# argsim/argsim

Measured on AMD Instinct MI355X. Metric: sentences/sec per ELBO step, higher is better.
Workload: dtype f32; 1 GPU; BASELINE configs[1]: 1xMI355X fp32, latent_dim 128, vocab 8k, seq_len 64, batch 256 per GPU; FULL synthetic Zipf batches, dim_emb 512, 3 layers, step 20000; global_batch=256, seq_len=64, parallelism=dp1, gru=persistent

## Files before the change

argsim_amd/csrc/kernels.h:

```cpp
#pragma once
#include <hip/hip_runtime.h>
#include <stdint.h>

#include "gemm_plan.h"

namespace avae {

struct GemmArgs {
    const float* A; const float* B; float* C; const float* bias;
    int M, N, K, lda, ldb, ldc;
    float alpha;
    int accumulate;
    int split_k;
    const int* dyn; int dyn_kind;
    int dyn_expect;
    int thin;
    const float* A2; const float* B2; float* C2; const float* bias2;
    float* slab = nullptr; size_t slab_floats = 0;
    unsigned short* c16 = nullptr;
    int nt8 = 1;
};
hipError_t gemm_f32(hipStream_t st, bool a_mc, bool b_nc, const GemmArgs& g);
hipError_t gemm_f32s(hipStream_t st, bool a_mc, bool b_nc, const GemmArgs& g);
hipError_t gemm_bf16_direct(hipStream_t st, bool a_mc, bool b_nc, const GemmArgs& g);
// ... 100 lines not shown
hipError_t embed_scatter_add2(hipStream_t st, float* dE, const int32_t* ids0, const float* dout0, int n0, const int32_t* ids1,
                              const float* dout1, int n1, int D, int V, int32_t* scratch);
bool id_groups_supported(int V);
inline size_t id_groups_ints(size_t n, size_t V) { return 4 * V + 2 + n + (n / 32 + V + 1) + 2 * V + 4; }
hipError_t id_groups_build(hipStream_t st, const int32_t* ids, int n, int V, int32_t* scratch, bool lists);
const int32_t* id_groups_rank(int32_t* scratch, int n, int V);
const int32_t* id_groups_uid(int32_t* scratch, int n, int V);
const int32_t* id_groups_count(int32_t* scratch, int n, int V);
hipError_t rank_rows(hipStream_t st, int32_t* out, const int32_t* ids, const int32_t* rank, int n, int V);
hipError_t rows_gather_ranked(hipStream_t st, float* dst, const float* src, const int32_t* ids, const int32_t* rank, int n, int W, int V);
hipError_t rows_group_sum(hipStream_t st, float* dst, const int32_t* ids, const float* src, int n, int W, int V, int32_t* scratch);
hipError_t rows_add_indexed(hipStream_t st, float* dst, const float* src, const int32_t* uid, const int32_t* nuniq, int n_max, int D);
inline size_t embed_scatter_scratch_ints(size_t n, size_t V) { return 4 * V + 2 + n + (n / 32 + V + 1); }
struct RowOrder { const int32_t* lens; int add, T, cpj; int32_t* perm; int32_t* slens; };
hipError_t row_order(hipStream_t st, const RowOrder* orders, int n, int Breal, int B, int S, int32_t* steps_sum = nullptr, int sum_rows = 0);
hipError_t rows_gather(hipStream_t st, float* dst, const float* src, const int32_t* idx, const int32_t* n_dev, int n_max, int D, const int32_t* map = nullptr);
hipError_t rows_expand(hipStream_t st, float* dst, const float* src, const int32_t* rank, int rows, int D, const int32_t* map = nullptr);
hipError_t pick_last(hipStream_t st, float* h, const float* hs, const int32_t* lens, int B, int W, const int32_t* map = nullptr);
hipError_t pick_last16(hipStream_t st, float* h, const unsigned short* hs16, const int32_t* lens, int B, int W, const int32_t* map = nullptr);
hipError_t pick_last_add(hipStream_t st, float* dhs, const float* d, const int32_t* lens, int B, int W, const int32_t* map = nullptr);
hipError_t row_map(hipStream_t st, const int32_t* lens, int add, int S, int B, int32_t* map, int32_t* nact, int32_t* count);
hipError_t zero_rows_dyn(hipStream_t st, float* X, const int32_t* count, int rows_max, int W);
hipError_t pick_last_bwd(hipStream_t st, float* dhs, const float* dh, const int32_t* lens, int S, int B, int W);

hipError_t latent_fwd(hipStream_t st, const float* mu, const float* lv, const float* eps_in, float* eps_out, float* z,
                      float* kld, int n, int train, uint64_t seed, float free_bits, float* acc);
hipError_t latent_bwd(hipStream_t st, const float* dz, const float* mu, const float* lv, const float* eps_used,
                      float* dmu, float* dlv, int B, int R, float coef, float free_bits);

struct CeArgs {
// ... 117 lines not shown
```

argsim_amd/csrc/model.cpp:

```cpp
#include "../../include/argsim_vae.h"
#include "kernels.h"

#include <fcntl.h>
#include <sys/file.h>
#include <unistd.h>

#include <algorithm>
#include <cmath>
#include <cstdio>
#include <cstring>
#include <string>
#include <vector>

using namespace avae;

namespace {

struct ParamEntry {
    std::string name;
    int64_t offset;
    int ndim;
    int64_t shape[4];
    int g16;
    int bucket;
// ... 12 lines not shown
    std::string err;
    std::vector<ParamEntry> params;
    int64_t numel = 0;
    std::vector<std::pair<int64_t, int64_t>> buckets;
    float *P = nullptr, *G = nullptr, *M = nullptr, *Vv = nullptr;
    int64_t step = 0;
    avae_grad_hook hook = nullptr; void* hook_user = nullptr;
    std::vector<int> hook_pending;
    int persistent = 1;
    bool first_step_checked = false;
    int gru_ablate = 0, gru_force_slow = 0, gru_stagger = 0, gru_item = 2;
    int skinny = 1;
    int score_plan[4] = {0, 0, 0, 0};
    const int* expect_ptr[3] = {nullptr, nullptr, nullptr}; int expect_val[3] = {0, 0, 0};
    int compact = 2;
    int skip_pad = 1;
    int shared_device = 0; int lock_fd = -1;
    int dyn_split = 1;
    int dyn_thin = 1;
    int enc_top1 = 1;
    int table_l1 = 1;
    int bf16_act = 1;
    int bf16_sv = 1;
    int bf16_tn = 1;
    int logits16 = 1;
    int bf16_nt8 = 1;
    int bf16_direct = 0;
    int gru_spec = 2;
    int bwd_rs = 2;
    int knn_chunk = 0;
// ... 75 lines not shown
    float *xlast, *gib, *svb, *dgib, *dghb, *dxl;
    float *hc, *ho, *logits;
    float *loss_samp, *errt_samp;
    float *dho, *dhc, *dhd[2], *dgi_d, *dgh_d, *dh0, *carry, *dh0sum, *dz, *dmu, *dlv, *dhpick;
    float *dhs[2], *dgi_e, *dgh_e, *demb_src, *demb_tgt;
    std::vector<unsigned short*> e_hs16, d_hd16, e_hp16[2], d_hp16;
    std::vector<char> act_e, act_d, acth_e, acth_d;
    std::vector<unsigned short*> x16_e, x16_d;
    const unsigned short* x16_kept_e(int i) const { return x16_valid ? x16_e[i] : nullptr; }
    const unsigned short* x16_kept_d(int i) const { return x16_valid ? x16_d[i] : nullptr; }
    bool x16_valid = false;
    unsigned short *dgi16_d, *dgh16_d, *dgi16_e, *dgh16_e;
    int32_t* scat;
    int32_t *grp_src, *grp_tgt;
    int32_t *tokrow_src, *tokrow_tgt;
    float* xbuf; size_t xbuf_floats;
    int32_t *ord_perm[3], *ord_slens[3]; int ord_T[3], ord_cpj[3]; bool ord_ok[3];
    int32_t *map_src, *nact_src, *nsrc; bool compact;
    int32_t *map_tgt, *nact_tgt, *ntgt; bool compact_d;
    int Bx;
    int bx_enc() const { return compact ? Bx : 0; }
    int bx_dec() const { return compact_d ? Bx : 0; }
};

struct Bump {
    char* base; size_t off = 0;
    template <class T> T* take(size_t n) {
        off = (off + 255) & ~(size_t)255;
        T* p = base ? reinterpret_cast<T*>(base + off) : nullptr;
        off += n * sizeof(T);
// ... 11 lines not shown
    return rows >= h->cfg.dim_tgt || (rows >= 1024 && phantom_batch(h, B));
}

void layout(avae_ctx* h, Bump& b, Ws& w, int B, int Ss, int St, bool train)
{
    const int D = h->cfg.dim_emb, V = h->cfg.dim_tgt, R = h->cfg.dim_rep, L = h->cfg.rnn_layers;
    const size_t T = St + 1, rs = (size_t)Ss * B, rt = T * B;
    w.src_tm = b.take<int32_t>(rs); w.lens_src = b.take<int32_t>(B); w.lens_tgt = b.take<int32_t>(B);
    w.lead = b.take<int32_t>(rt); w.gold = b.take<int32_t>(rt); w.rank = b.take<int32_t>(rt);
    w.cidx = b.take<int32_t>(rt); w.ntok = b.take<int32_t>(4 + kPrepChunks); w.pred = b.take<int32_t>(rt);
    w.emb_src = b.take<float>(rs * D); w.emb_tgt = b.take<float>(rt * D);
    const bool tab_s = use_table(h, (int)rs, B), tab_t = use_table(h, (int)rt, B);
    w.ew = b.take<float>(tab_s ? (size_t)V * 6 * D : (tab_t ? (size_t)V * 3 * D : 0));
    w.grp_src = b.take<int32_t>(tab_s ? id_groups_ints(rs, V) : 0); w.grp_tgt = b.take<int32_t>(tab_t ? id_groups_ints(rt, V) : 0);
    w.tokrow_src = b.take<int32_t>(tab_s ? rs : 0); w.tokrow_tgt = b.take<int32_t>(tab_t ? rt : 0);
    w.e_gi.resize(L); w.e_hs.resize(L);
    for (int d = 0; d < 2; ++d) { w.e_sv[d].resize(L); w.e_hp[d].resize(L); }
    w.d_gi.resize(L); w.d_hd.resize(L); w.d_sv.resize(L); w.d_hp.resize(L);
    w.e_hs16.assign(L, nullptr); w.d_hd16.assign(L, nullptr); w.e_hp16[0].assign(L, nullptr); w.e_hp16[1].assign(L, nullptr); w.d_hp16.assign(L, nullptr);
    w.act_e.assign(L, 0); w.act_d.assign(L, 0); w.acth_e.assign(L, 0); w.acth_d.assign(L, 0);
    if (train && h->cfg.compute_dtype == 1 && h->bf16_act && h->bf16_tn && D % 8 == 0)
        for (int i = 0; i < L; ++i) {
            w.e_hs16[i] = b.take<unsigned short>(rs * 2 * D); w.e_hp16[0][i] = b.take<unsigned short>(rs * D); w.e_hp16[1][i] = b.take<unsigned short>(rs * D);
            if (i < L - 1) w.d_hd16[i] = b.take<unsigned short>(rt * D);
            w.d_hp16[i] = b.take<unsigned short>(rt * D);
        }
    w.x16_e.assign(L, nullptr); w.x16_d.assign(L, nullptr);
    w.x16_valid = train && h->cfg.compute_dtype == 1 && h->bf16_tn && !h->bf16_direct && D % 8 == 0;
    if (w.x16_valid)
        for (int i = 1; i < L; ++i) { w.x16_e[i] = b.take<unsigned short>(rs * 2 * D); w.x16_d[i] = b.take<unsigned short>(rt * D); }
// ... 310 lines not shown
{
    if (h->gru_spec != 2) return h->gru_spec;
    return expected_fill(h) < 0.60 ? 1 : 0;
}

static void gru_common(avae_ctx* h, const Ws& w, GruArgs& a, int njobs, int S, int B, int ldg, int ldh, const int32_t* lens, int Bx)
{
    const int D = h->cfg.dim_emb;
    a.njobs = njobs; a.S = S; a.B = B; a.D = D; a.ldg = ldg; a.ldh = ldh; a.lens = lens;
    a.Bx = Bx;
    gru_geometry(D, njobs, B, &a.G, &a.rows_per_group);
    a.p_begin = 0; a.p_end = S; a.counters = h->counters; a.err = h->errw; a.ablate = h->gru_ablate; a.force_slow = h->gru_force_slow;
    a.bf16 = h->cfg.compute_dtype == 1 && h->gru_bf16; a.stagger = h->gru_stagger; a.item_pipeline = h->gru_item;
    a.xbuf = w.xbuf; a.xbuf_floats = w.xbuf_floats; a.stamps = reinterpret_cast<unsigned long long*>(h->errw + 16); a.bwd_rs = h->bwd_rs != 0;
}
int build_row_orders(avae_ctx* h, Ws& w, int B, int Ss, int T, bool with_dec, bool with_enc = true)
{
    if (!h->skip_pad || !h->persistent || w.Bx % 16) return 0;
    if (w.Bx != B && !h->compact) return 0;
    const int D = h->cfg.dim_emb;
    RowOrder ord[3]; int n = 0, which[3];
    auto want = [&](int k, int njobs, int S, int ldg, int ldh, const int32_t* lens, int add) {
        GruArgs a{};
        gru_common(h, w, a, njobs, S, B, ldg, ldh, lens, w.Bx);
        const GruPlan p = gru_plan(a, true, true);
        if (p.form != GruForm::team) return;
        ord[n] = RowOrder{lens, add, p.T, p.cpj, w.ord_perm[k], w.ord_slens[k]};
        which[n++] = k; w.ord_T[k] = p.T; w.ord_cpj[k] = p.cpj;
    };
    if (with_enc) want(0, 2, Ss, 6 * D, 2 * D, w.lens_src, 0);
    if (with_enc && top_one_step(h)) want(1, 1, Ss, 6 * D, 2 * D, w.lens_src, 0);
    if (with_dec) want(2, 1, T, 3 * D, D, w.lens_tgt, 1);
    if (!n) return 0;
    const bool hint = which[0] == 0 && h->compact == 2;
    if (hint && !h->hint_host) {
        int32_t* hp = nullptr;
        if (hipHostMalloc(reinterpret_cast<void**>(&hp), 64, hipHostMallocDefault) == hipSuccess) { hp[0] = -1; hp[1] = 0; h->hint_host = hp; }
    }
    h->hint_dev = reinterpret_cast<int32_t*>(h->errw + 100);
    hipError_t e = row_order(h->stream, ord, n, B, w.Bx, std::max(Ss, T), hint ? h->hint_dev : nullptr, Ss * B);
    if (e == hipErrorInvalidValue) return 0;
    AV_CHECK(e);
    if (hint && h->hint_host) {
        AV_CHECK(hipMemcpyAsync(const_cast<int32_t*>(h->hint_host), h->hint_dev, 2 * sizeof(int32_t), hipMemcpyDeviceToHost, h->stream));
    }
    for (int i = 0; i < n; ++i) w.ord_ok[which[i]] = true;
    return 0;
}
static bool both_team_bf16(avae_ctx* h, const GruArgs& a, bool train)
{
    return train && a.bf16 && gru_plan(a, true, h->persistent != 0).full() && gru_plan(a, false, h->persistent != 0).full();
}
static void attach_sv16(avae_ctx* h, GruArgs& a, bool train) { a.sv16 = h->bf16_sv && both_team_bf16(h, a, train); }
static void attach_order(avae_ctx* h, const Ws& w, GruArgs& a, bool fwd, int k)
{
    const GruPlan p = gru_plan(a, fwd, h->persistent != 0);
// ... 51 lines not shown
int run_encoder(avae_ctx* h, Ws& w, int B, int Ss, bool save)
{
    const int D = h->cfg.dim_emb, V = h->cfg.dim_tgt, L = h->cfg.rnn_layers;
    const int rs = Ss * B;
    const bool table = use_table(h, rs, B);
    h->cnt_src = table ? id_groups_count(w.grp_src, rs, V) : nullptr;
    const int32_t* const cdyn = w.compact ? w.nsrc : nullptr;
    const int32_t* const cmap = w.compact ? w.map_src : nullptr;
    if (!table) AV_CHECK(embed_gather(h->stream, h->P + h->oE, w.src_tm, w.emb_src, rs, D, V));
    const float* x = w.emb_src; int In = D;
    for (int i = 0; i < L; ++i) {
        const GruP& p = h->enc[i];
        const bool top1 = i == L - 1 && top_one_step(h);
        if (i == 0 && table) {
            const int32_t* cnt = id_groups_count(w.grp_src, rs, V);
            AV_CHECK(id_groups_build(h->stream, w.src_tm, rs, V, w.grp_src, save));
            AV_CHECK(rows_gather(h->stream, w.emb_src, h->P + h->oE, id_groups_uid(w.grp_src, rs, V), cnt, std::min(V, rs), D));
            AV_TRY(gemm(h, nt(w.emb_src, D, h->P + p.W, D, w.ew, 6 * D, std::min(V, rs), 6 * D, D).biased(h->P + p.bW).rows(cnt)));
        } else if (i > 0 && w.act_e[i - 1]) {
            AV_TRY(gemm_bf16_pre(h, nt(nullptr, In, h->P + p.W, In, w.e_gi[i], 6 * D, rs, top1 ? 3 * D : 6 * D, In).a16(w.e_hs16[i - 1]).biased(h->P + p.bW).rows(cdyn)));
        } else {
        AV_TRY(gemm(h, nt(x, In, h->P + p.W, In, w.e_gi[i], 6 * D, rs, top1 ? 3 * D : 6 * D, In).biased(h->P + p.bW).rows(cdyn).keep(save ? w.x16_e[i] : nullptr)));
        }
        GruArgs a{};
        gru_common(h, w, a, top1 ? 1 : 2, Ss, B, 6 * D, 2 * D, w.lens_src, w.bx_enc());
        const bool table0 = i == 0 && table, indirect = table0 && gru_plan(a, true, h->persistent != 0).form == GruForm::team;
        if (indirect) AV_CHECK(rank_rows(h->stream, w.tokrow_src, w.src_tm, id_groups_rank(w.grp_src, rs, V), rs, V));
        else if (table0) AV_CHECK(rows_gather_ranked(h->stream, w.e_gi[0], w.ew, w.src_tm, id_groups_rank(w.grp_src, rs, V), rs, 6 * D, V));
        for (int d = 0; d < a.njobs; ++d) {
            GruJob& j = a.job[d];
            j.gi = (indirect ? w.ew : w.e_gi[i]) + d * 3 * D;
            j.gi_rows = indirect ? w.tokrow_src : nullptr;
            j.R = h->P + p.R + (int64_t)d * 3 * D * D;
            j.bR = h->P + p.bR + d * 3 * D;
            j.h0 = nullptr;
            j.hs = w.e_hs[i] + d * D;
            j.sv = save ? w.e_sv[d][i] : nullptr;
            j.hp = save ? w.e_hp[d][i] : nullptr;
            j.reverse = d;
        }
        attach_sv16(h, a, save);
        if (w.e_hs16[i] && tn16_ok(h, 3 * D, D) && both_team_bf16(h, a, save)) {
// ... 36 lines not shown

int run_decoder_rnn(avae_ctx* h, Ws& w, int B, int T, const float* state_in, int64_t state_stride, bool save, const int32_t* ids0 = nullptr, bool compact = false,
                    const int32_t* share_rows = nullptr, int share_n = 0)
{
    const int32_t* const cdyn = compact ? w.ntgt : nullptr;
    const int32_t* const cmap = compact ? w.map_tgt : nullptr;
    const int D = h->cfg.dim_emb, L = h->cfg.rnn_layers;
    const int rt = T * B;
    const float* x = w.emb_tgt;
    h->cnt_tgt = ids0 ? id_groups_count(w.grp_tgt, rt, h->cfg.dim_tgt) : nullptr;
    for (int i = 0; i < L; ++i) {
        const GruP& p = h->dec[i];
        if (i == 0 && ids0) {
            const int V = h->cfg.dim_tgt;
            const int32_t* cnt = id_groups_count(w.grp_tgt, rt, V);
            AV_CHECK(id_groups_build(h->stream, ids0, rt, V, w.grp_tgt, save));
            AV_CHECK(rows_gather(h->stream, w.emb_tgt, h->P + h->oE, id_groups_uid(w.grp_tgt, rt, V), cnt, std::min(V, rt), D));
            AV_TRY(gemm(h, nt(w.emb_tgt, D, h->P + p.W, D, w.ew, 3 * D, std::min(V, rt), 3 * D, D).biased(h->P + p.bW).rows(cnt)));
        } else if (i == 0 && share_rows) {
            AV_TRY(gemm(h, nt(x, D, h->P + p.W, D, w.d_gi[0], 3 * D, share_n, 3 * D, D).biased(h->P + p.bW)));
        } else if (i > 0 && w.act_d[i - 1]) {
            AV_TRY(gemm_bf16_pre(h, nt(nullptr, D, h->P + p.W, D, w.d_gi[i], 3 * D, rt, 3 * D, D).a16(w.d_hd16[i - 1]).biased(h->P + p.bW).rows(cdyn)));
        } else {
        AV_TRY(gemm(h, nt(x, D, h->P + p.W, D, w.d_gi[i], 3 * D, rt, 3 * D, D).biased(h->P + p.bW).rows(cdyn).keep(save ? w.x16_d[i] : nullptr)));
        }
        GruArgs a{};
        gru_common(h, w, a, 1, T, B, 3 * D, D, nullptr, compact ? w.Bx : 0);
        GruJob& j = a.job[0];
        const bool table0 = i == 0 && ids0, indirect = table0 && gru_plan(a, true, h->persistent != 0).form == GruForm::team;
        if (indirect) AV_CHECK(rank_rows(h->stream, w.tokrow_tgt, ids0, id_groups_rank(w.grp_tgt, rt, h->cfg.dim_tgt), rt, h->cfg.dim_tgt));
        else if (table0) AV_CHECK(rows_gather_ranked(h->stream, w.d_gi[0], w.ew, ids0, id_groups_rank(w.grp_tgt, rt, h->cfg.dim_tgt), rt, 3 * D, h->cfg.dim_tgt));
        j.gi = indirect ? w.ew : w.d_gi[i]; j.gi_rows = indirect ? w.tokrow_tgt : nullptr;
        if (i == 0 && share_rows) j.gi_rows = share_rows;
        j.R = h->P + p.R; j.bR = h->P + p.bR;
        j.h0 = state_in + state_stride * i;
        j.hs = w.d_hd[i];
        j.sv = save ? w.d_sv[i] : nullptr;
        j.hp = save ? w.d_hp[i] : nullptr;
        j.reverse = 0;
        attach_sv16(h, a, save);
        if (w.d_hp16[i] && tn16_ok(h, 3 * D, D) && both_team_bf16(h, a, save)) {
            if (i < L - 1) { w.act_d[i] = 1; j.hs16 = w.d_hd16[i]; }
            w.acth_d[i] = 1; j.hp16 = w.d_hp16[i];
        }
        if (T > 1) attach_order(h, w, a, true, 2);
// ... 8 lines not shown
}

int run_logits_ce(avae_ctx* h, Ws& w, int rt, bool train, float inv_n);

int forward(avae_ctx* h, Ws& w, const int32_t* src, const int32_t* tgt, int B, int Ss, int St, bool train,
            uint64_t seed, const uint8_t* keep_mask, const float* eps, float inv_n)
{
    const int D = h->cfg.dim_emb, V = h->cfg.dim_tgt, R = h->cfg.dim_rep;
    const int T = St + 1, rt = T * B;
    Sched sc = schedule(h);
    PrepArgs p{};
    p.src = src; p.tgt = tgt; p.B = B; p.Ss = Ss; p.St = St; p.eos = h->cfg.eos; p.bos = h->cfg.bos;
    p.train = train ? 1 : 0; p.keepwd = sc.keepwd; p.seed = seed; p.keep_mask = keep_mask;
    p.src_tm = w.src_tm; p.lens_src = w.lens_src; p.lens_tgt = w.lens_tgt; p.lead = w.lead; p.gold = w.gold;
    p.rank = w.rank; p.cidx = w.cidx; p.ntok = w.ntok; p.chunk_counts = w.ntok + 4; p.zero2 = nullptr;
    AV_CHECK(prep_ids(h->stream, p));
    AV_TRY(build_row_orders(h, w, B, Ss, T, true));
    AV_TRY(build_compact(h, w, B, Ss, T, train));
    AV_TRY(run_encoder(h, w, B, Ss, train));
    AV_TRY(run_latent(h, w, B, train, seed, eps));
    AV_TRY(gemm(h, nn(w.z, R, h->P + h->oWex, D, w.h0, D, B, D, R).biased(h->P + h->oBex).batch_rows()));
    if (use_table(h, rt, B)) AV_TRY(run_decoder_rnn(h, w, B, T, w.h0, 0, train, w.lead, w.compact_d));
    else {
        AV_CHECK(embed_gather(h->stream, h->P + h->oE, w.lead, w.emb_tgt, rt, D, V));
        AV_TRY(run_decoder_rnn(h, w, B, T, w.h0, 0, train));
    }
    AV_TRY(run_logits_ce(h, w, rt, train, inv_n));
    float beta = h->cfg.kl_beta;
    AV_CHECK(finalize_losses(h->stream, h->losses, w.loss_samp, w.ntok, rt, w.kld, B * R, h->cfg.free_bits, 1.f / ((float)B * R), sc.anneal * beta));
    return 0;
}

// ... 564 lines not shown
    if (!strcmp(key, "gru_force_slow")) { h->gru_force_slow = value; return 0; }
    if (!strcmp(key, "gru_bf16")) { h->gru_bf16 = value != 0; return 0; }
    if (!strcmp(key, "bwd_rs")) { h->bwd_rs = value; return 0; }
    if (!strcmp(key, "dyn_split")) { h->dyn_split = value != 0; return 0; }
    if (!strcmp(key, "shared_device")) { h->shared_device = value != 0; return 0; }
    if (!strcmp(key, "gru_spec")) { h->gru_spec = value; return 0; }
    if (!strcmp(key, "bf16_nt8")) { h->bf16_nt8 = value != 0; return 0; }
    if (!strcmp(key, "logits16")) { h->logits16 = value != 0; return 0; }
    if (!strcmp(key, "bf16_direct")) { h->bf16_direct = value != 0; return 0; }
    if (!strcmp(key, "bf16_tn")) { h->bf16_tn = value != 0; return 0; }
    if (!strcmp(key, "bf16_sv")) { h->bf16_sv = value != 0; return 0; }
    if (!strcmp(key, "bf16_act")) { h->bf16_act = value != 0; return 0; }
    if (!strcmp(key, "table_l1")) { h->table_l1 = value != 0; return 0; }
    if (!strcmp(key, "enc_top1")) { h->enc_top1 = value != 0; return 0; }
    if (!strcmp(key, "dyn_thin")) { h->dyn_thin = value != 0; return 0; }
    if (!strcmp(key, "skip_pad")) { h->skip_pad = value != 0; return 0; }
    if (!strcmp(key, "compact")) { h->compact = value; return 0; }
    if (!strcmp(key, "skinny")) { h->skinny = value; return 0; }
    if (!strcmp(key, "knn_chunk")) { if (value < 0) return fail(h, "knn_chunk must be >= 0"); h->knn_chunk = value; return 0; }
    if (!strcmp(key, "gru_ablate")) {
        if (value && !gru_diag_build()) return fail(h, "gru_ablate needs the diagnostic build of libargsim_vae.so (make -C argsim_amd/csrc DIAG=1)");
        h->gru_ablate = value; return 0;
    }
    if (!strcmp(key, "timing")) { h->timing = value; h->timing_on = value; h->stamps_used = 0; return 0; }
    if (!strcmp(key, "timing_pause")) { h->timing = value ? 0 : h->timing_on; return 0; }
    return fail(h, "unknown option");
}
static int dyn_fraction(avae_ctx* h, const avae_ctx::Stamp& s, std::vector<std::pair<const int*, int>>& seen, double* f)
{
    *f = 1.0;
// ... 172 lines not shown
}
int avae_debug_op(avae_handle h, const char* op, void* const* p, const int64_t* i, const float* f)
{
    if (!h || !op || !p || !i || !f) return 1;
    const std::string o(op);
    hipStream_t st = h->stream;
    auto F = [&](int k) { return static_cast<float*>(p[k]); };
    auto I = [&](int k) { return static_cast<int32_t*>(p[k]); };
    if (o == "prep_ids") {
        PrepArgs a{};
        a.src = I(0); a.tgt = I(1); a.keep_mask = static_cast<const uint8_t*>(p[2]); a.src_tm = I(3); a.lens_src = I(4); a.lens_tgt = I(5);
        a.lead = I(6); a.gold = I(7); a.rank = I(8); a.cidx = I(9); a.ntok = I(10); a.zero2 = F(11); a.chunk_counts = I(12);
        a.B = (int)i[0]; a.Ss = (int)i[1]; a.St = (int)i[2]; a.eos = (int)i[3]; a.bos = (int)i[4]; a.train = (int)i[5]; a.seed = (uint64_t)i[6];
        a.keepwd = f[0];
        AV_CHECK(prep_ids(st, a));
    } else if (o == "embed_gather") AV_CHECK(embed_gather(st, F(0), I(1), F(2), (int)i[0], (int)i[1], (int)i[2]));
    else if (o == "embed_scatter_add2") AV_CHECK(embed_scatter_add2(st, F(0), I(1), F(2), (int)i[0], I(3), F(4), (int)i[1], (int)i[2], (int)i[3], I(5)));
    else if (o == "id_groups_build") AV_CHECK(id_groups_build(st, I(0), (int)i[0], (int)i[1], I(1), i[2] != 0));
    else if (o == "rank_rows") AV_CHECK(rank_rows(st, I(0), I(1), I(2), (int)i[0], (int)i[1]));
    else if (o == "rows_gather_ranked") AV_CHECK(rows_gather_ranked(st, F(0), F(1), I(2), I(3), (int)i[0], (int)i[1], (int)i[2]));
    else if (o == "rows_group_sum") AV_CHECK(rows_group_sum(st, F(0), I(1), F(2), (int)i[0], (int)i[1], (int)i[2], I(3)));
    else if (o == "rows_add_indexed") AV_CHECK(rows_add_indexed(st, F(0), F(1), I(2), I(3), (int)i[0], (int)i[1]));
    else if (o == "rows_gather") AV_CHECK(rows_gather(st, F(0), F(1), I(2), I(3), (int)i[0], (int)i[1], I(4)));
    else if (o == "rows_expand") AV_CHECK(rows_expand(st, F(0), F(1), I(2), (int)i[0], (int)i[1], I(3)));
    else if (o == "zero_rows_dyn") AV_CHECK(zero_rows_dyn(st, F(0), I(1), (int)i[0], (int)i[1]));
    else if (o == "zero_fill") AV_CHECK(zero_fill(st, p[0], (size_t)i[0]));
    else if (o == "row_order") {
        RowOrder ro[4];
        const int n = (int)i[0];
        for (int k = 0; k < std::min(n, 4); ++k) ro[k] = RowOrder{I(3 * k), (int)i[5 + 3 * k], (int)i[6 + 3 * k], (int)i[7 + 3 * k], I(3 * k + 1), I(3 * k + 2)};
// ... 570 lines not shown
```

argsim_amd/csrc/ops.hip:

```cpp
#include <algorithm>
#include "kernels.h"
#include "sample_dev.h"

namespace avae {


__device__ __forceinline__ bool prep_kept(const PrepArgs& p, int i)
{
    const int t = i / p.B, b = i - t * p.B;
    return t == 0 || p.tgt[(size_t)b * p.St + t - 1] != p.eos;
}
__device__ __forceinline__ int block_sum256(int v, int* red)
{
#pragma unroll
    for (int o = 32; o > 0; o >>= 1) v += __shfl_xor(v, o);
    if ((threadIdx.x & 63) == 0) red[threadIdx.x >> 6] = v;
    __syncthreads();
    const int s = red[0] + red[1] + red[2] + red[3];
    __syncthreads();
    return s;
}
__global__ __launch_bounds__(256) void prep_ids_kernel(PrepArgs p, int per, int nchunks)
{
    __shared__ int red[4];
// ... 258 lines not shown
        if (n0 > 0) hipLaunchKernelGGL(embed_scatter_atomic_kernel, dim3(std::min((n0 + 3) / 4, 4096)), dim3(256), 0, st, dE, ids0, dout0, n0, D, V);
        if (n1 > 0) hipLaunchKernelGGL(embed_scatter_atomic_kernel, dim3(std::min((n1 + 3) / 4, 4096)), dim3(256), 0, st, dE, ids1, dout1, n1, D, V);
        return hipGetLastError();
    }
    Scatter2 a{dE, ids0, dout0, n0, ids1, dout1, n1, D, V, scratch, scratch + V, scratch + 2 * V, scratch + 3 * V + 1, scratch + 4 * V + 2, scratch + 4 * V + 2 + n, nullptr, nullptr, nullptr};
    hipError_t e = zero_fill(st, scratch, sizeof(int32_t) * 2 * (size_t)V);
    if (e != hipSuccess) return e;
    const int blocks = (n + kScatterTok - 1) / kScatterTok;
    hipLaunchKernelGGL(scatter_hist_kernel, dim3(blocks), dim3(256), 0, st, a);
    hipLaunchKernelGGL(scatter_scan_kernel, dim3(1), dim3(1024), 0, st, a);
    hipLaunchKernelGGL(scatter_fill_kernel, dim3(blocks), dim3(256), 0, st, a);
    hipLaunchKernelGGL(scatter_reduce_kernel, dim3(std::min((n / 4 + V + 3) / 4, 4096)), dim3(256), 0, st, a);
    return hipGetLastError();
}

static Scatter2 id_groups_view(const int32_t* ids, int n, int V, int32_t* scratch)
{
    int32_t* rank = scratch + 4 * (size_t)V + 2 + n + ((size_t)n / kScatterSeg + V + 1);
    return Scatter2{nullptr, ids, nullptr, n, nullptr, nullptr, 0, 0, V, scratch, scratch + V, scratch + 2 * V, scratch + 3 * V + 1,
                    scratch + 4 * V + 2, scratch + 4 * (size_t)V + 2 + n, rank, rank + V, rank + 2 * (size_t)V};
}
const int32_t* id_groups_rank(int32_t* scratch, int n, int V) { return id_groups_view(nullptr, n, V, scratch).rank; }
const int32_t* id_groups_uid(int32_t* scratch, int n, int V) { return id_groups_view(nullptr, n, V, scratch).uid; }
const int32_t* id_groups_count(int32_t* scratch, int n, int V) { return id_groups_view(nullptr, n, V, scratch).nuniq; }
bool id_groups_supported(int V) { return V <= kScatterLdsV; }
hipError_t id_groups_build(hipStream_t st, const int32_t* ids, int n, int V, int32_t* scratch, bool lists)
{
    if (n <= 0 || V > kScatterLdsV) return hipErrorInvalidValue;
    Scatter2 a = id_groups_view(ids, n, V, scratch);
    hipError_t e = zero_fill(st, scratch, sizeof(int32_t) * 2 * (size_t)V);
    if (e != hipSuccess) return e;
// ... 158 lines not shown
        int rank = 0;
        for (int c = 0; c < B; ++c) { const int v = steps[c]; rank += (v > mine) || (v == mine && c < b); }
        const int g = rank >> 4, w = g % o.cpj, jj = g / o.cpj;
        const int slot = (((w + (jj / o.T) * o.cpj) * o.T + jj % o.T) << 4) + (rank & 15);
        o.perm[slot] = b;
        o.slens[slot] = mine;
    }
}
hipError_t row_order(hipStream_t st, const RowOrder* orders, int n, int Breal, int B, int S, int32_t* steps_sum, int sum_rows)
{
    if (n <= 0) return hipSuccess;
    if (n > 3 || B % 16 || B < Breal || (size_t)B * 4 > 64 * 1024) return hipErrorInvalidValue;
    RowOrders ro{};
    for (int i = 0; i < n; ++i) ro.o[i] = orders[i];
    hipLaunchKernelGGL(row_order_kernel, dim3(n), dim3(1024), (size_t)B * sizeof(int), st, ro, Breal, B, S, steps_sum, sum_rows);
    return hipGetLastError();
}

__global__ __launch_bounds__(256) void row_map_local_kernel(const int32_t* __restrict__ lens, int add, int B, int32_t* __restrict__ map, int32_t* __restrict__ nact)
{
    __shared__ int scan[256];
    __shared__ int base_s;
    const int t = blockIdx.x, tid = threadIdx.x;
    if (tid == 0) base_s = 0;
    __syncthreads();
    for (int b0 = 0; b0 < B; b0 += 256) {
        const int b = b0 + tid;
        const int act = (b < B && t < lens[b] + add) ? 1 : 0;
        scan[tid] = act;
        __syncthreads();
// ... 709 lines not shown
        if (to_g16) dst[i] = src[nat * cols + col];
        else dst[nat * cols + col] = src[i];
    }
}
hipError_t g16_permute(hipStream_t st, float* dst, const float* src, int D, int cols, bool to_g16)
{
    int64_t total = (int64_t)3 * D * cols;
    hipLaunchKernelGGL(g16_permute_kernel, dim3((unsigned)((total + 255) / 256 < 2048 ? (total + 255) / 256 : 2048)), dim3(256), 0, st, dst, src, D, cols, to_g16 ? 1 : 0);
    return hipGetLastError();
}

__global__ __launch_bounds__(1024) void finalize_losses_kernel(float* losses, const float* __restrict__ loss_samp, const int32_t* n_dev, int n_max,
                                                               const float* __restrict__ kld, int nk, float free_bits, float inv_br, float anneal)
{
    __shared__ float sh[2][1024];
    const int tid = threadIdx.x, n = min(n_max, *n_dev);
    float sg = 0.f, sk = 0.f;
    for (int i = tid; i < n; i += 1024) sg += loss_samp[i];
    for (int i = tid; i < nk; i += 1024) sk += fmaxf(kld[i], free_bits);
    sh[0][tid] = sg; sh[1][tid] = sk;
    __syncthreads();
    for (int o = 512; o > 0; o >>= 1) {
        if (tid < o) { sh[0][tid] += sh[0][tid + o]; sh[1][tid] += sh[1][tid + o]; }
        __syncthreads();
    }
    if (tid == 0) {
        const float gen = sh[0][0] / (float)max(n, 1), kl = sh[1][0] * inv_br;
        losses[0] = gen; losses[1] = kl; losses[2] = anneal * kl + gen;
    }
}
hipError_t finalize_losses(hipStream_t st, float* losses, const float* loss_samp, const int32_t* n_dev, int n_max,
                           const float* kld, int nk, float free_bits, float inv_br, float anneal)
{
    hipLaunchKernelGGL(finalize_losses_kernel, dim3(1), dim3(1024), 0, st, losses, loss_samp, n_dev, n_max, kld, nk, free_bits, inv_br, anneal);
// ... 5 lines not shown
```

Before: 15590 sentences/sec.

## Fuse id prep, row ordering and id-group building into one prep kernel

Adds a single two-block prep_step kernel, one block per side (source and target). It runs the id transpose and length computation, the lead/rank compaction, the row-order permutation and the id-group/tokrow construction, including an in-LDS radix sort for the token lists. This replaces several separate small launches (prep_ids, row_order, id_groups_build, rank_rows) with one, cutting launch and serialization overhead in the per-step preamble. It also reorders and unrolls the loss-finalize reduction loads. The trade-off is doing all of this prep work on only two workgroups.

```diff
diff --git a/argsim_amd/csrc/kernels.h b/argsim_amd/csrc/kernels.h
--- a/argsim_amd/csrc/kernels.h
+++ b/argsim_amd/csrc/kernels.h
@@ -138,6 +138,16 @@
 inline size_t embed_scatter_scratch_ints(size_t n, size_t V) { return 4 * V + 2 + n + (n / 32 + V + 1); }
 struct RowOrder { const int32_t* lens; int add, T, cpj; int32_t* perm; int32_t* slens; };
 hipError_t row_order(hipStream_t st, const RowOrder* orders, int n, int Breal, int B, int S, int32_t* steps_sum = nullptr, int sum_rows = 0);
+struct PrepStep {
+    PrepArgs p;
+    int V, lists, nord, Bx, S, sum_rows;
+    int groups[2];
+    int32_t* grp[2]; int32_t* tokrow[2]; int32_t* tmp[2];
+    RowOrder ord[3];
+    int32_t* steps_sum;
+};
+bool prep_step_supported(int B, int Bx, int Ss, int St, int V);
+hipError_t prep_step(hipStream_t st, const PrepStep& a);
 hipError_t rows_gather(hipStream_t st, float* dst, const float* src, const int32_t* idx, const int32_t* n_dev, int n_max, int D, const int32_t* map = nullptr);
 hipError_t rows_expand(hipStream_t st, float* dst, const float* src, const int32_t* rank, int rows, int D, const int32_t* map = nullptr);
 hipError_t pick_last(hipStream_t st, float* h, const float* hs, const int32_t* lens, int B, int W, const int32_t* map = nullptr);
diff --git a/argsim_amd/csrc/model.cpp b/argsim_amd/csrc/model.cpp
--- a/argsim_amd/csrc/model.cpp
+++ b/argsim_amd/csrc/model.cpp
@@ -50,6 +50,7 @@
     int score_plan[4] = {0, 0, 0, 0};
     const int* expect_ptr[3] = {nullptr, nullptr, nullptr}; int expect_val[3] = {0, 0, 0};
     int compact = 2;
+    int prep_fused = 1;
     int skip_pad = 1;
     int shared_device = 0; int lock_fd = -1;
     int dyn_split = 1;
@@ -155,6 +156,8 @@
     int32_t* scat;
     int32_t *grp_src, *grp_tgt;
     int32_t *tokrow_src, *tokrow_tgt;
+    int32_t* prep_tmp[2];
+    bool prep_done = false;
     float* xbuf; size_t xbuf_floats;
     int32_t *ord_perm[3], *ord_slens[3]; int ord_T[3], ord_cpj[3]; bool ord_ok[3];
     int32_t *map_src, *nact_src, *nsrc; bool compact;
@@ -196,6 +199,7 @@
     w.ew = b.take<float>(tab_s ? (size_t)V * 6 * D : (tab_t ? (size_t)V * 3 * D : 0));
     w.grp_src = b.take<int32_t>(tab_s ? id_groups_ints(rs, V) : 0); w.grp_tgt = b.take<int32_t>(tab_t ? id_groups_ints(rt, V) : 0);
     w.tokrow_src = b.take<int32_t>(tab_s ? rs : 0); w.tokrow_tgt = b.take<int32_t>(tab_t ? rt : 0);
+    w.prep_tmp[0] = b.take<int32_t>(tab_s ? rs : 0); w.prep_tmp[1] = b.take<int32_t>(tab_t ? rt : 0);
     w.e_gi.resize(L); w.e_hs.resize(L);
     for (int d = 0; d < 2; ++d) { w.e_sv[d].resize(L); w.e_hp[d].resize(L); }
     w.d_gi.resize(L); w.d_hd.resize(L); w.d_sv.resize(L); w.d_hp.resize(L);
@@ -536,10 +540,12 @@
     a.bf16 = h->cfg.compute_dtype == 1 && h->gru_bf16; a.stagger = h->gru_stagger; a.item_pipeline = h->gru_item;
     a.xbuf = w.xbuf; a.xbuf_floats = w.xbuf_floats; a.stamps = reinterpret_cast<unsigned long long*>(h->errw + 16); a.bwd_rs = h->bwd_rs != 0;
 }
-int build_row_orders(avae_ctx* h, Ws& w, int B, int Ss, int T, bool with_dec, bool with_enc = true)
-{
-    if (!h->skip_pad || !h->persistent || w.Bx % 16) return 0;
-    if (w.Bx != B && !h->compact) return 0;
+int build_row_orders(avae_ctx* h, Ws& w, int B, int Ss, int T, bool with_dec, bool with_enc = true, PrepStep* fused = nullptr)
+{
+    if (fused) fused->nord = 0;
+    auto none = [&]() { if (fused) AV_CHECK(prep_step(h->stream, *fused)); return 0; };
+    if (!h->skip_pad || !h->persistent || w.Bx % 16) return none();
+    if (w.Bx != B && !h->compact) return none();
     const int D = h->cfg.dim_emb;
     RowOrder ord[3]; int n = 0, which[3];
     auto want = [&](int k, int njobs, int S, int ldg, int ldh, const int32_t* lens, int add) {
@@ -553,15 +559,21 @@
     if (with_enc) want(0, 2, Ss, 6 * D, 2 * D, w.lens_src, 0);
     if (with_enc && top_one_step(h)) want(1, 1, Ss, 6 * D, 2 * D, w.lens_src, 0);
     if (with_dec) want(2, 1, T, 3 * D, D, w.lens_tgt, 1);
-    if (!n) return 0;
+    if (!n) return none();
     const bool hint = which[0] == 0 && h->compact == 2;
     if (hint && !h->hint_host) {
         int32_t* hp = nullptr;
         if (hipHostMalloc(reinterpret_cast<void**>(&hp), 64, hipHostMallocDefault) == hipSuccess) { hp[0] = -1; hp[1] = 0; h->hint_host = hp; }
     }
     h->hint_dev = reinterpret_cast<int32_t*>(h->errw + 100);
-    hipError_t e = row_order(h->stream, ord, n, B, w.Bx, std::max(Ss, T), hint ? h->hint_dev : nullptr, Ss * B);
-    if (e == hipErrorInvalidValue) return 0;
+    hipError_t e;
+    if (fused) {
+        fused->nord = n; fused->Bx = w.Bx; fused->S = std::max(Ss, T); fused->steps_sum = hint ? h->hint_dev : nullptr; fused->sum_rows = Ss * B;
+        for (int i = 0; i < n; ++i) fused->ord[i] = ord[i];
+        e = prep_step(h->stream, *fused);
+    } else
+    e = row_order(h->stream, ord, n, B, w.Bx, std::max(Ss, T), hint ? h->hint_dev : nullptr, Ss * B);
+    if (e == hipErrorInvalidValue && !fused) return 0;
     AV_CHECK(e);
     if (hint && h->hint_host) {
         AV_CHECK(hipMemcpyAsync(const_cast<int32_t*>(h->hint_host), h->hint_dev, 2 * sizeof(int32_t), hipMemcpyDeviceToHost, h->stream));
@@ -643,7 +655,7 @@
         const bool top1 = i == L - 1 && top_one_step(h);
         if (i == 0 && table) {
             const int32_t* cnt = id_groups_count(w.grp_src, rs, V);
-            AV_CHECK(id_groups_build(h->stream, w.src_tm, rs, V, w.grp_src, save));
+            if (!w.prep_done) AV_CHECK(id_groups_build(h->stream, w.src_tm, rs, V, w.grp_src, save));
             AV_CHECK(rows_gather(h->stream, w.emb_src, h->P + h->oE, id_groups_uid(w.grp_src, rs, V), cnt, std::min(V, rs), D));
             AV_TRY(gemm(h, nt(w.emb_src, D, h->P + p.W, D, w.ew, 6 * D, std::min(V, rs), 6 * D, D).biased(h->P + p.bW).rows(cnt)));
         } else if (i > 0 && w.act_e[i - 1]) {
@@ -654,7 +666,8 @@
         GruArgs a{};
         gru_common(h, w, a, top1 ? 1 : 2, Ss, B, 6 * D, 2 * D, w.lens_src, w.bx_enc());
         const bool table0 = i == 0 && table, indirect = table0 && gru_plan(a, true, h->persistent != 0).form == GruForm::team;
-        if (indirect) AV_CHECK(rank_rows(h->stream, w.tokrow_src, w.src_tm, id_groups_rank(w.grp_src, rs, V), rs, V));
+        if (indirect && w.prep_done) {}
+        else if (indirect) AV_CHECK(rank_rows(h->stream, w.tokrow_src, w.src_tm, id_groups_rank(w.grp_src, rs, V), rs, V));
         else if (table0) AV_CHECK(rows_gather_ranked(h->stream, w.e_gi[0], w.ew, w.src_tm, id_groups_rank(w.grp_src, rs, V), rs, 6 * D, V));
         for (int d = 0; d < a.njobs; ++d) {
             GruJob& j = a.job[d];
@@ -721,7 +734,7 @@
         if (i == 0 && ids0) {
             const int V = h->cfg.dim_tgt;
             const int32_t* cnt = id_groups_count(w.grp_tgt, rt, V);
-            AV_CHECK(id_groups_build(h->stream, ids0, rt, V, w.grp_tgt, save));
+            if (!w.prep_done) AV_CHECK(id_groups_build(h->stream, ids0, rt, V, w.grp_tgt, save));
             AV_CHECK(rows_gather(h->stream, w.emb_tgt, h->P + h->oE, id_groups_uid(w.grp_tgt, rt, V), cnt, std::min(V, rt), D));
             AV_TRY(gemm(h, nt(w.emb_tgt, D, h->P + p.W, D, w.ew, 3 * D, std::min(V, rt), 3 * D, D).biased(h->P + p.bW).rows(cnt)));
         } else if (i == 0 && share_rows) {
@@ -735,7 +748,8 @@
         gru_common(h, w, a, 1, T, B, 3 * D, D, nullptr, compact ? w.Bx : 0);
         GruJob& j = a.job[0];
         const bool table0 = i == 0 && ids0, indirect = table0 && gru_plan(a, true, h->persistent != 0).form == GruForm::team;
-        if (indirect) AV_CHECK(rank_rows(h->stream, w.tokrow_tgt, ids0, id_groups_rank(w.grp_tgt, rt, h->cfg.dim_tgt), rt, h->cfg.dim_tgt));
+        if (indirect && w.prep_done) {}
+        else if (indirect) AV_CHECK(rank_rows(h->stream, w.tokrow_tgt, ids0, id_groups_rank(w.grp_tgt, rt, h->cfg.dim_tgt), rt, h->cfg.dim_tgt));
         else if (table0) AV_CHECK(rows_gather_ranked(h->stream, w.d_gi[0], w.ew, ids0, id_groups_rank(w.grp_tgt, rt, h->cfg.dim_tgt), rt, 3 * D, h->cfg.dim_tgt));
         j.gi = indirect ? w.ew : w.d_gi[i]; j.gi_rows = indirect ? w.tokrow_tgt : nullptr;
         if (i == 0 && share_rows) j.gi_rows = share_rows;
@@ -774,8 +788,19 @@
     p.train = train ? 1 : 0; p.keepwd = sc.keepwd; p.seed = seed; p.keep_mask = keep_mask;
     p.src_tm = w.src_tm; p.lens_src = w.lens_src; p.lens_tgt = w.lens_tgt; p.lead = w.lead; p.gold = w.gold;
     p.rank = w.rank; p.cidx = w.cidx; p.ntok = w.ntok; p.chunk_counts = w.ntok + 4; p.zero2 = nullptr;
+    struct Reset { bool& f; ~Reset() { f = false; } } reset{w.prep_done};
+    w.prep_done = h->prep_fused && prep_step_supported(B, std::max(w.Bx, B), Ss, St, V);
+    if (w.prep_done) {
+        PrepStep ps{};
+        ps.p = p; ps.V = V; ps.lists = train ? 1 : 0;
+        ps.groups[0] = use_table(h, Ss * B, B); ps.groups[1] = use_table(h, rt, B);
+        ps.grp[0] = w.grp_src; ps.grp[1] = w.grp_tgt; ps.tokrow[0] = w.tokrow_src; ps.tokrow[1] = w.tokrow_tgt;
+        ps.tmp[0] = w.prep_tmp[0]; ps.tmp[1] = w.prep_tmp[1];
+        AV_TRY(build_row_orders(h, w, B, Ss, T, true, true, &ps));
+    } else {
     AV_CHECK(prep_ids(h->stream, p));
     AV_TRY(build_row_orders(h, w, B, Ss, T, true));
+    }
     AV_TRY(build_compact(h, w, B, Ss, T, train));
     AV_TRY(run_encoder(h, w, B, Ss, train));
     AV_TRY(run_latent(h, w, B, train, seed, eps));
@@ -1370,6 +1395,7 @@
     if (!strcmp(key, "table_l1")) { h->table_l1 = value != 0; return 0; }
     if (!strcmp(key, "enc_top1")) { h->enc_top1 = value != 0; return 0; }
     if (!strcmp(key, "dyn_thin")) { h->dyn_thin = value != 0; return 0; }
+    if (!strcmp(key, "prep_fused")) { h->prep_fused = value != 0; return 0; }
     if (!strcmp(key, "skip_pad")) { h->skip_pad = value != 0; return 0; }
     if (!strcmp(key, "compact")) { h->compact = value; return 0; }
     if (!strcmp(key, "skinny")) { h->skinny = value; return 0; }
@@ -1572,6 +1598,20 @@
         a.B = (int)i[0]; a.Ss = (int)i[1]; a.St = (int)i[2]; a.eos = (int)i[3]; a.bos = (int)i[4]; a.train = (int)i[5]; a.seed = (uint64_t)i[6];
         a.keepwd = f[0];
         AV_CHECK(prep_ids(st, a));
+    } else if (o == "prep_step") {
+        PrepStep s{};
+        PrepArgs& a = s.p;
+        a.src = I(0); a.tgt = I(1); a.keep_mask = static_cast<const uint8_t*>(p[2]); a.src_tm = I(3); a.lens_src = I(4); a.lens_tgt = I(5);
+        a.lead = I(6); a.gold = I(7); a.rank = I(8); a.cidx = I(9); a.ntok = I(10); a.zero2 = F(11); a.chunk_counts = I(12);
+        a.B = (int)i[0]; a.Ss = (int)i[1]; a.St = (int)i[2]; a.eos = (int)i[3]; a.bos = (int)i[4]; a.train = (int)i[5]; a.seed = (uint64_t)i[6];
+        a.keepwd = f[0];
+        s.V = (int)i[7]; s.lists = (int)i[8]; s.groups[0] = (int)i[9]; s.groups[1] = (int)i[10]; s.nord = (int)i[11]; s.Bx = (int)i[12]; s.S = (int)i[13];
+        s.sum_rows = (int)i[14];
+        for (int k = 0; k < 2; ++k) { s.grp[k] = I(13 + 3 * k); s.tokrow[k] = I(14 + 3 * k); s.tmp[k] = I(15 + 3 * k); }
+        const int n = std::min(std::max(s.nord, 0), 3);
+        for (int k = 0; k < n; ++k) s.ord[k] = RowOrder{I(19 + 3 * k), (int)i[15 + 3 * k], (int)i[16 + 3 * k], (int)i[17 + 3 * k], I(20 + 3 * k), I(21 + 3 * k)};
+        s.steps_sum = I(19 + 3 * n);
+        AV_CHECK(prep_step(st, s));
     } else if (o == "embed_gather") AV_CHECK(embed_gather(st, F(0), I(1), F(2), (int)i[0], (int)i[1], (int)i[2]));
     else if (o == "embed_scatter_add2") AV_CHECK(embed_scatter_add2(st, F(0), I(1), F(2), (int)i[0], I(3), F(4), (int)i[1], (int)i[2], (int)i[3], I(5)));
     else if (o == "id_groups_build") AV_CHECK(id_groups_build(st, I(0), (int)i[0], (int)i[1], I(1), i[2] != 0));
diff --git a/argsim_amd/csrc/ops.hip b/argsim_amd/csrc/ops.hip
--- a/argsim_amd/csrc/ops.hip
+++ b/argsim_amd/csrc/ops.hip
@@ -296,7 +296,7 @@
     return hipGetLastError();
 }
 
-static Scatter2 id_groups_view(const int32_t* ids, int n, int V, int32_t* scratch)
+__host__ __device__ static Scatter2 id_groups_view(const int32_t* ids, int n, int V, int32_t* scratch)
 {
     int32_t* rank = scratch + 4 * (size_t)V + 2 + n + ((size_t)n / kScatterSeg + V + 1);
     return Scatter2{nullptr, ids, nullptr, n, nullptr, nullptr, 0, 0, V, scratch, scratch + V, scratch + 2 * V, scratch + 3 * V + 1,
@@ -485,6 +485,182 @@
     RowOrders ro{};
     for (int i = 0; i < n; ++i) ro.o[i] = orders[i];
     hipLaunchKernelGGL(row_order_kernel, dim3(n), dim3(1024), (size_t)B * sizeof(int), st, ro, Breal, B, S, steps_sum, sum_rows);
+    return hipGetLastError();
+}
+
+constexpr int kPrepStepTok = 32768, kPrepStepB = 2048;
+static_assert(kScatterLdsV <= (1 << 14) && kPrepStepTok <= (1 << 16), "prep_step packs (id, token) into 30 bits");
+__device__ __forceinline__ int clamp_id(int id, int V) { return id < 0 ? 0 : (id >= V ? V - 1 : id); }
+__device__ __forceinline__ unsigned long long match_digit(int d, bool valid)
+{
+    unsigned long long peers = __ballot(valid);
+#pragma unroll
+    for (int bit = 0; bit < 7; ++bit) {
+        const bool s = (d >> bit) & 1;
+        const unsigned long long b = __ballot(valid && s);
+        peers &= s ? b : ~b;
+    }
+    return peers;
+}
+template <int PASS>
+__device__ __forceinline__ void prep_step_radix(const int32_t* ids, int V, int n, const int32_t* in, int32_t* out, int* mat, int* wsum)
+{
+    const int tid = threadIdx.x, lane = tid & 63, wave = tid >> 6;
+    const int chunks = (n + 63) >> 6, cpw = (chunks + 15) >> 4, c0 = min(chunks, wave * cpw), c1 = min(chunks, c0 + cpw);
+    mat[tid] = 0; mat[tid + 1024] = 0;
+    __syncthreads();
+    for (int c = c0; c < c1; ++c) {
+        const int i = c * 64 + lane;
+        const bool valid = i < n;
+        const int key = !valid ? 0 : (PASS == 0 ? ((clamp_id(ids[i], V) << 16) | i) : in[i]);
+        const int d = (key >> (16 + 7 * PASS)) & 127;
+        const unsigned long long peers = match_digit(d, valid);
+        if (valid && lane == __ffsll((long long)peers) - 1) mat[d * 16 + wave] += __popcll(peers);
+    }
+    __syncthreads();
+    {
+        const int v0 = mat[2 * tid], v1 = mat[2 * tid + 1];
+        const int e = block_scan1024(v0 + v1, wsum) - v0 - v1;
+        mat[2 * tid] = e; mat[2 * tid + 1] = e + v0;
+    }
+    __syncthreads();
+    for (int c = c0; c < c1; ++c) {
+        const int i = c * 64 + lane;
+        const bool valid = i < n;
+        const int key = !valid ? 0 : (PASS == 0 ? ((clamp_id(ids[i], V) << 16) | i) : in[i]);
+        const int d = (key >> (16 + 7 * PASS)) & 127;
+        const unsigned long long peers = match_digit(d, valid);
+        const int leader = __ffsll((long long)peers) - 1;
+        int base = 0;
+        if (valid && lane == leader) { base = mat[d * 16 + wave]; mat[d * 16 + wave] = base + __popcll(peers); }
+        base = __shfl(base, leader & 63, 64);
+        if (valid) out[base + __popcll(peers & ((1ull << lane) - 1ull))] = PASS == 0 ? key : (key & 0xffff);
+    }
+    __syncthreads();
+}
+__device__ __forceinline__ void prep_step_groups(const int32_t* ids, int n, int V, int32_t* scratch, int32_t* tokrow, int32_t* tmp, bool lists,
+                                                 int* lc, int* mat, int* wsum)
+{
+    const Scatter2 a = id_groups_view(ids, n, V, scratch);
+    const int tid = threadIdx.x;
+    for (int i = tid; i < V; i += 1024) lc[i] = 0;
+    __syncthreads();
+    for (int t = tid; t < n; t += 1024) atomicAdd(&lc[clamp_id(ids[t], V)], 1);
+    __syncthreads();
+    {
+        const int per = (V + 1023) / 1024, beg = min(V, tid * per), end = min(V, beg + per);
+        int tok = 0, seg = 0, uni = 0;
+        for (int i = beg; i < end; ++i) { const int c = lc[i]; tok += c; seg += (c + kScatterSeg - 1) / kScatterSeg; uni += c > 0; }
+        const int itok = block_scan1024(tok, wsum), iseg = block_scan1024(seg, wsum), iuni = block_scan1024(uni, wsum);
+        int rt = itok - tok, rs = iseg - seg, ru = iuni - uni;
+        for (int i = beg; i < end; ++i) {
+            const int c = lc[i];
+            a.cnt[i] = c; a.off[i] = rt; a.segoff[i] = rs;
+            rt += c;
+            for (int k = (c + kScatterSeg - 1) / kScatterSeg; k > 0; --k) a.segid[rs++] = i;
+            a.rank[i] = c > 0 ? ru : -1; lc[i] = c > 0 ? ru : -1;
+            if (c > 0) a.uid[ru++] = i;
+        }
+        if (tid == 1023) { a.off[V] = itok; a.segoff[V] = iseg; a.nuniq[0] = iuni; }
+    }
+    __syncthreads();
+    if (tokrow) for (int t = tid; t < n; t += 1024) tokrow[t] = lc[clamp_id(ids[t], V)];
+    if (lists) {
+        prep_step_radix<0>(ids, V, n, nullptr, tmp, mat, wsum);
+        prep_step_radix<1>(ids, V, n, tmp, a.list, mat, wsum);
+    }
+}
+__device__ __forceinline__ void prep_step_order(const RowOrder& o, int Breal, int B, int S, int* steps, int32_t* steps_sum, int sum_rows)
+{
+    for (int b = threadIdx.x; b < B; b += 1024) steps[b] = b < Breal ? min(max(o.lens[b] + o.add, 1), S) : 1;
+    __syncthreads();
+    if (steps_sum && threadIdx.x < 64) {
+        int v = 0;
+        for (int b = threadIdx.x; b < Breal; b += 64) v += steps[b];
+        for (int off = 32; off > 0; off >>= 1) v += __shfl_xor(v, off, 64);
+        if (threadIdx.x == 0) { steps_sum[0] = v; steps_sum[1] = sum_rows; }
+    }
+    for (int b = threadIdx.x; b < B; b += 1024) {
+        const int mine = steps[b];
+        int rank = 0;
+        for (int c = 0; c < B; ++c) { const int v = steps[c]; rank += (v > mine) || (v == mine && c < b); }
+        const int g = rank >> 4, w = g % o.cpj, jj = g / o.cpj;
+        const int slot = (((w + (jj / o.T) * o.cpj) * o.T + jj % o.T) << 4) + (rank & 15);
+        o.perm[slot] = b;
+        o.slens[slot] = mine;
+    }
+    __syncthreads();
+}
+__global__ __launch_bounds__(1024) void prep_step_kernel(PrepStep a)
+{
+    __shared__ int lc[kScatterLdsV];
+    __shared__ int mat[2048];
+    __shared__ int wsum[16];
+    const PrepArgs& p = a.p;
+    const int tid = threadIdx.x, lane = tid & 63, wave = tid >> 6, side = blockIdx.x, B = p.B;
+    const int32_t* lens = side == 0 ? p.lens_src : p.lens_tgt;
+    if (side == 0) {
+        for (int b = wave; b < B; b += 16) {
+            int ls = 0;
+            for (int s = lane; s < p.Ss; s += 64) { const int v = p.src[(size_t)b * p.Ss + s]; ls += v != p.eos; p.src_tm[(size_t)s * B + b] = v; }
+#pragma unroll
+            for (int o = 32; o > 0; o >>= 1) ls += __shfl_xor(ls, o);
+            if (lane == 0) p.lens_src[b] = ls;
+        }
+        if (tid < 2 && p.zero2) p.zero2[tid] = 0.f;
+    } else {
+        const int total = (p.St + 1) * B;
+        for (int b = wave; b < B; b += 16) {
+            int lt = 0;
+            for (int s = lane; s < p.St; s += 64) { const int v = p.tgt[(size_t)b * p.St + s]; if (v != p.eos) lt = s + 1; p.gold[(size_t)s * B + b] = v; }
+#pragma unroll
+            for (int o = 32; o > 0; o >>= 1) lt = max(lt, __shfl_xor(lt, o));
+            if (lane == 0) { p.lens_tgt[b] = lt; p.gold[(size_t)p.St * B + b] = p.eos; }
+        }
+        __syncthreads();
+        for (int i = tid; i < total; i += 1024) {
+            int lead = p.bos;
+            if (i >= B) {
+                lead = p.gold[i - B];
+                if (p.train) {
+                    const int j = i - B;
+                    const bool keep = p.keep_mask ? p.keep_mask[j] != 0 : uniform01(p.seed, 1, j) < p.keepwd;
+                    if (!keep) lead = 0;
+                }
+            }
+            p.lead[i] = lead;
+        }
+        const int ept = (total + 1023) / 1024, beg = min(total, tid * ept), end = min(total, beg + ept);
+        int cnt = 0;
+        for (int i = beg; i < end; ++i) cnt += i < B || p.gold[i - B] != p.eos;
+        const int incl = block_scan1024(cnt, wsum);
+        int run = incl - cnt;
+        for (int i = beg; i < end; ++i) {
+            const bool m = i < B || p.gold[i - B] != p.eos;
+            p.rank[i] = m ? run : -1;
+            if (m) p.cidx[run++] = i;
+        }
+        if (tid == 1023) p.ntok[0] = incl;
+    }
+    __syncthreads();
+    for (int k = 0; k < a.nord; ++k)
+        if (a.ord[k].lens == lens) prep_step_order(a.ord[k], B, a.Bx, a.S, mat, k == 0 ? a.steps_sum : nullptr, a.sum_rows);
+    if (a.groups[side])
+        prep_step_groups(side == 0 ? p.src_tm : p.lead, side == 0 ? p.Ss * B : (p.St + 1) * B, a.V, a.grp[side], a.tokrow[side], a.tmp[side], a.lists != 0,
+                         lc, mat, wsum);
+}
+bool prep_step_supported(int B, int Bx, int Ss, int St, int V)
+{
+    return B > 0 && Ss > 0 && St > 0 && V > 0 && V <= kScatterLdsV && (long long)Ss * B <= kPrepStepTok && ((long long)St + 1) * B <= kPrepStepTok &&
+           Bx >= B && Bx <= kPrepStepB;
+}
+hipError_t prep_step(hipStream_t st, const PrepStep& a)
+{
+    if (!prep_step_supported(a.p.B, a.nord ? a.Bx : a.p.B, a.p.Ss, a.p.St, a.V) || a.nord < 0 || a.nord > 3) return hipErrorInvalidValue;
+    if (a.nord && a.Bx % 16) return hipErrorInvalidValue;
+    for (int k = 0; k < a.nord; ++k) if (a.ord[k].lens != a.p.lens_src && a.ord[k].lens != a.p.lens_tgt) return hipErrorInvalidValue;
+    for (int s = 0; s < 2; ++s) if (a.groups[s] && (!a.grp[s] || (a.lists && !a.tmp[s]))) return hipErrorInvalidValue;
+    hipLaunchKernelGGL(prep_step_kernel, dim3(2), dim3(1024), 0, st, a);
     return hipGetLastError();
 }
 
@@ -1224,10 +1400,23 @@
                                                                const float* __restrict__ kld, int nk, float free_bits, float inv_br, float anneal)
 {
     __shared__ float sh[2][1024];
-    const int tid = threadIdx.x, n = min(n_max, *n_dev);
+    const int tid = threadIdx.x, n_in = *n_dev;
     float sg = 0.f, sk = 0.f;
-    for (int i = tid; i < n; i += 1024) sg += loss_samp[i];
-    for (int i = tid; i < nk; i += 1024) sk += fmaxf(kld[i], free_bits);
+    for (int i0 = tid; i0 < nk; i0 += 16 * 1024) {
+        float v[16];
+#pragma unroll
+        for (int u = 0; u < 16; ++u) { const int i = i0 + u * 1024; v[u] = i < nk ? kld[i] : 0.f; }
+#pragma unroll
+        for (int u = 0; u < 16; ++u) if (i0 + u * 1024 < nk) sk += fmaxf(v[u], free_bits);
+    }
+    const int n = min(n_max, n_in);
+    for (int i0 = tid; i0 < n; i0 += 16 * 1024) {
+        float v[16];
+#pragma unroll
+        for (int u = 0; u < 16; ++u) { const int i = i0 + u * 1024; v[u] = i < n ? loss_samp[i] : 0.f; }
+#pragma unroll
+        for (int u = 0; u < 16; ++u) if (i0 + u * 1024 < n) sg += v[u];
+    }
     sh[0][tid] = sg; sh[1][tid] = sk;
     __syncthreads();
     for (int o = 512; o > 0; o >>= 1) {
```

Result: no change. 15570 sentences/sec (-0.2%).
